# NetSys/demi

Hardware: AMD Instinct MI355X
Metric: candidate schedules evaluated/sec on Raft-5 fuzz (RandomScheduler executions) (higher is better)
Workload: dtype u8

## Files before the change

demi_amd/_native.py:

```python
import ctypes as C
import os

from . import types as T

_HERE = os.path.dirname(os.path.abspath(__file__))
LIB_PATH = os.path.join(_HERE, "libdemi_gpu.so")

EXPORTS = ["demi_ctx_create", "demi_ctx_destroy", "demi_last_error", "demi_version", "demi_model_load",
           "demi_trace_load", "demi_random_explore", "demi_random_explore_dev", "demi_random_get_trace", "demi_collect_violations_dev",
           "demi_replay_load", "demi_replay_batch", "demi_replay_batch_dev", "demi_dpor_load", "demi_dpor_batch", "demi_dpor_explore", "demi_random_explore_violations", "demi_random_get_trace_carried",
           "demi_replay_removal_batch", "demi_replay_get_kept", "demi_replay_recorded_len", "demi_ddmin", "demi_dpor_set_traces", "demi_model_specialize", "demi_model_is_specialized", "demi_model_code_id",
           "demi_specialize_check", "demi_specialize_source", "demi_specialize_source_k1", "demi_provenance_prune", "demi_device_probe", "demi_device_probe_mix", "demi_calib_rw", "demi_random_explore_flagged", "demi_collect_flagged_dev", "demi_random_explore_submit", "demi_random_explore_wait", "demi_trace_len",
           "demi_comm_unique_id", "demi_comm_create", "demi_comm_create_host", "demi_comm_destroy", "demi_comm_rank",
           "demi_comm_allgather_dev", "demi_random_explore_sharded", "demi_replay_batch_sharded", "demi_abi_version", "demi_replay_externals_len", "demi_edit_distance_dpor_ddmin", "demi_dpor_explored", "demi_random_ddmin", "demi_random_explore_candidates", "demi_ext_payload_areas",
           "demi_replay_wildcard_load", "demi_replay_wildcard_batch", "demi_replay_wildcard_get_trace",
           "demi_replay_wildcard_candidates", "demi_wildcard_ddmin",
           "demi_fuzz_stride", "demi_fuzz_generate", "demi_random_explore_tests", "demi_fuzz_campaign",
           "demi_fuzz_generate_fields", "demi_random_explore_tests_areas", "demi_fuzz_campaign_fields",
           "demi_fuzz_launch_summary", "demi_fuzz_launch_summary_row", "demi_fuzz_campaign_pipelined",
           "demi_replay_removal_round", "demi_minimize_internals", "demi_replay_wildcard_round", "demi_minimize_wildcards",
           "demi_replay_batch_submit", "demi_replay_batch_wait",
           "demi_dpor_wildcard_batch", "demi_wildcard_dpor_test"]

_lib = None
# ... 131 lines not shown
                                            C.c_void_p, C.c_void_p, C.c_void_p, C.c_void_p]
    L.demi_random_explore_tests_areas.argtypes = [C.c_void_p, C.c_uint64, C.c_void_p, C.c_void_p, C.c_void_p, C.c_uint32, C.c_uint32, C.c_uint32,
                                                  C.POINTER(T.Limits), C.c_void_p, C.c_void_p]
    L.demi_fuzz_campaign_fields.argtypes = [C.c_void_p, C.POINTER(T.FuzzParams), C.POINTER(T.FuzzFieldGen), C.POINTER(T.FuzzCampaignParams),
                                            C.POINTER(T.Limits), C.c_void_p, C.c_void_p, C.c_uint32, C.POINTER(T.FuzzCampaignResult)]
    L.demi_fuzz_launch_summary.argtypes = [C.c_void_p, C.c_void_p, C.c_void_p, C.c_uint32, C.c_uint32, C.POINTER(T.FuzzSummary)]
    L.demi_fuzz_launch_summary_row.argtypes = [C.c_void_p, C.c_void_p, C.c_void_p, C.c_uint32]
    L.demi_fuzz_campaign_pipelined.argtypes = [C.c_void_p, C.POINTER(T.FuzzParams), C.POINTER(T.FuzzFieldGen), C.POINTER(T.FuzzCampaignParams),
                                               C.POINTER(T.FuzzPipelineParams), C.POINTER(T.Limits), C.c_void_p, C.c_void_p, C.c_uint32,
                                               C.POINTER(T.FuzzCampaignResult), C.POINTER(T.FuzzPipelineStats)]
    L.demi_replay_removal_round.argtypes = [C.c_void_p, C.c_void_p, C.c_void_p, C.c_uint32, C.POINTER(T.Limits), C.c_void_p,
                                            C.POINTER(T.RemovalRoundResult)]
    L.demi_minimize_internals.argtypes = [C.c_void_p, C.POINTER(T.Limits), C.POINTER(T.IntminParams), C.c_void_p, C.c_uint32,
                                          C.POINTER(C.c_uint32), C.c_void_p, C.c_uint32, C.c_void_p, C.c_uint32, C.POINTER(T.IntminStats)]
    L.demi_replay_wildcard_round.argtypes = [C.c_void_p, C.c_void_p, C.c_void_p, C.c_uint32, C.POINTER(T.Limits), C.c_void_p,
                                             C.POINTER(T.WildcardRoundResult)]
    L.demi_minimize_wildcards.argtypes = [C.c_void_p, C.POINTER(T.Limits), C.POINTER(T.WcminParams), C.c_void_p, C.c_uint32,
                                          C.POINTER(C.c_uint32), C.c_void_p, C.c_uint32, C.c_void_p, C.c_uint32, C.POINTER(T.WcminStats)]
    for name in EXPORTS:
        fn = getattr(L, name)
        assert fn.argtypes is not None or name in ("demi_version",), "no argtypes for %s" % name
    _lib = L
    return L


def specialize_check(model_struct):
    log = C.create_string_buffer(4096)
    n = lib().demi_specialize_check(C.byref(model_struct), log, len(log))
    if n < 0:
        raise DemiError(n, log.value.decode(errors="replace"))
    return int(n), log.value.decode()


def specialize_source(model_struct, k1=False):
    buf = C.create_string_buffer(1 << 20)
    n = (lib().demi_specialize_source_k1 if k1 else lib().demi_specialize_source)(C.byref(model_struct), buf, len(buf))
    if n < 0:
        raise DemiError(n, buf.value.decode(errors="replace"))
    return buf.value.decode()


class Context:

    def __init__(self, device=0):
        self._h = C.c_void_p()
        rc = lib().demi_ctx_create(device, C.byref(self._h))
        if rc != 0:
            raise DemiError(rc, "demi_ctx_create failed (no MI355X visible? the GPU path has no CPU fallback)")
        self.device = device

    def close(self):
        if self._h:
            lib().demi_ctx_destroy(self._h)
            self._h = C.c_void_p()

    def __del__(self):
        try:
            self.close()
        except Exception:
            pass

    def _check(self, rc):
        if rc != 0:
            raise DemiError(rc, lib().demi_last_error(self._h).decode())

    def model_load(self, model_struct):
        self._check(lib().demi_model_load(self._h, C.byref(model_struct)))

    def model_specialize(self, enable=True):
# ... 715 lines not shown
```

demi_amd/csrc/demi_gpu.hip:

```cpp
#include <hip/hip_runtime.h>

#include <cstdarg>
#include <cstdio>
#include <cstring>
#include <algorithm>
#include <memory>
#include <new>
#include <queue>
#include <string>
#include <type_traits>
#include <unordered_map>
#include <unordered_set>
#include <vector>
#include <chrono>

#include "../../include/demi_gpu.h"
#include "knobs.hpp"
#include "devbuf.hpp"
#include "k1_random_explore.hpp"
#include "k2_replay.hpp"
#include "k2_removal_round.hpp"
#include "k2_wildcard.hpp"
#include "k2_wildcard_cand.hpp"
#include "k2_wildcard_round.hpp"
// ... 610 lines not shown
           h.n_timer_types, h.timer_types, (unsigned long long)h.tix_packed, h.n_msg_types);
  src = defs + src;
  if (h.inv_kind & DEMI_INV_PROGRAM) src = "#define DEMI_JIT_INV_PROG 1\n" + src;
  if (h.wide) src = "#define DEMI_WIDE 1\n" + src;
  if (is_big(h)) {
    uint32_t type_of_tix = 0;
    for (uint32_t t = 0; t < h.n_msg_types; t++) if ((h.timer_types >> t) & 1u) type_of_tix |= t << (5u * (h.meta[t] >> 8));
    src = "#define DEMI_BIG 1\n#define DEMI_JIT_TYPE_OF_TIX " + std::to_string(type_of_tix) + "u\n" + src;
  }
  if (kernel == JK_K3W) src = "#define DEMI_K3_DECLS_ONLY 1\n" + src;
  src = demi_jit::tq_defines(h) + src;
  src = demi_jit::init_hits_define(h) + src;
  if (h.npay > 2) src = "#define DEMI_JIT_NPAY " + std::to_string(h.npay) + "\n" + src;
  if (h.arr_len) src = "#define DEMI_JIT_ARR_LEN " + std::to_string(h.arr_len) + "u\n" + src;
  {
    bool crash = false, rnd = false;
    for (uint32_t pc = 0; pc < h.code_len; pc++) { crash |= (h.code[pc] & 0xFFu) == DEMI_OP_CRASH; rnd |= (h.code[pc] & 0x3Fu) == DEMI_OP_RND; }
    if (!crash) src = "#define DEMI_JIT_NO_CRASH 1\n" + src;
    if (!rnd) src = "#define DEMI_JIT_NO_RND 1\n" + src;
  }
  if (const char* d = demi_host::knob("DEMI_JIT_DEFINES")) {
    std::string extra, item;
    for (const char* c = d;; c++) {
      if (*c == ';' || *c == '\0') {
        if (!item.empty()) { const size_t eq = item.find('='); extra += "#define " + (eq == std::string::npos ? item : item.substr(0, eq) + " " + item.substr(eq + 1)) + "\n"; }
        item.clear();
        if (*c == '\0') break;
      } else item += *c;
    }
    src = extra + src;
  }
  if (const long x = demi_host::knob_int("DEMI_JIT_K1_WAVES_PER_EU", 1, 8, 0))
    src = "#define DEMI_K1_MIN_WAVES_PER_EU " + std::to_string(x) + "\n" + src;
  src += demi_jit::generate_vm(h, jk_is_k1(kernel) && !jk_k1_records(kernel) && !demi_host::knob("DEMI_JIT_NO_FX_SCHED"));
  src += "#define DEMI_VM_RUN vm_run_jit\n#include \"";
  src += kJit[kernel].include;
  src += "\"\n";
  if (kJit[kernel].args) src += std::string("template __global__ void ") + kJit[kernel].name + "(const " + kJit[kernel].args + ");\n";
  return src;
}

static int jit_compile(demi_ctx* ctx, const DevModel& h, int kernel, std::vector<char>& image, std::string& name) {
#ifdef DEMI_NO_JIT_SOURCES
  return fail(ctx, DEMI_ERR_DEVICE, "specialisation failed: this library was built without the embedded kernel sources "
                                    "(build it with __graft_entry__.build())");
#endif
  static demi_jit::Rtc rtc;
  std::vector<demi_jit::Header> headers(kJitHeaders, kJitHeaders + sizeof(kJitHeaders) / sizeof(kJitHeaders[0]));
  std::vector<std::string> lowered;
  std::string err;
  std::string source = jit_source(h, kernel);
#ifdef DEMI_K1_PHASES
  source = "#define DEMI_K1_PHASES 1\n" + source;
#endif
  if (const char* dump = demi_host::knob("DEMI_JIT_DUMP_SRC")) {
    if (FILE* f = fopen((std::string(dump) + "." + std::to_string(kernel)).c_str(), "w")) { fputs(source.c_str(), f); fclose(f); }
  }
  const char* level = (jk_is_k1(kernel) && !jk_k1_records(kernel)) ? "-Os" : "-O3";
  if (!demi_jit::compile(rtc, source, headers, {kJit[kernel].name}, image, lowered, err, level))
    return fail(ctx, DEMI_ERR_DEVICE, "specialisation failed: %s", err.c_str());
  name = lowered[0];
  if (const char* dump = demi_host::knob("DEMI_JIT_DUMP")) {
    if (FILE* f = fopen((std::string(dump) + "." + std::to_string(kernel)).c_str(), "wb")) { fwrite(image.data(), 1, image.size(), f); fclose(f); }
  }
  return DEMI_OK;
}

static uint64_t code_object_text_hash(const std::vector<char>& image) {
  const unsigned char* b = reinterpret_cast<const unsigned char*>(image.data());
  size_t lo = 0, hi = image.size();
  auto rd = [&](size_t off, int bytes) -> uint64_t {
    uint64_t v = 0;
    for (int i = 0; i < bytes; i++) v |= (uint64_t)b[off + i] << (8 * i);
    return v;
  };
  if (image.size() > 64 && b[0] == 0x7F && b[1] == 'E' && b[2] == 'L' && b[3] == 'F' && b[4] == 2) {
    const uint64_t shoff = rd(0x28, 8), shentsize = rd(0x3A, 2), shnum = rd(0x3C, 2), shstrndx = rd(0x3E, 2);
    if (shentsize >= 64 && shstrndx < shnum && shoff + shnum * shentsize <= image.size()) {
      const uint64_t stroff = rd(shoff + shstrndx * shentsize + 0x18, 8), strsize = rd(shoff + shstrndx * shentsize + 0x20, 8);
      for (uint64_t i = 0; i < shnum; i++) {
        const uint64_t sh = shoff + i * shentsize, name = rd(sh, 4), off = rd(sh + 0x18, 8), size = rd(sh + 0x20, 8);
        if (name + 6 <= strsize && stroff + name + 6 <= image.size() && !memcmp(b + stroff + name, ".text", 6) &&
            off + size <= image.size()) { lo = off; hi = off + size; }
      }
    }
  }
  uint64_t h = 0xCBF29CE484222325ULL;
  for (size_t i = lo; i < hi; i++) h = (h ^ b[i]) * 0x100000001B3ULL;
  return h ? h : 1;
}

static int jit_load(demi_ctx* ctx, int k) {
  std::vector<char> image;
  std::string name;
  int rc = jit_compile(ctx, ctx->hmodel, k, image, name);
  if (rc) return rc;
  if (k == JK_K1) ctx->jit_code_id = code_object_text_hash(image);
  if (jk_is_k1(k) && !jk_k1_records(k)) ctx->jit_k1_fxq_slots = demi_jit::k1_fxq_slots(ctx->hmodel, !demi_host::knob("DEMI_JIT_NO_FX_SCHED"));
  HIP_TRY(ctx, hipSetDevice(ctx->device));
  hipError_t e = hipModuleLoadData(&ctx->jit_module[k], image.data());
  if (e != hipSuccess) { ctx->jit_module[k] = nullptr; return fail(ctx, DEMI_ERR_DEVICE, "hipModuleLoadData: %s", hipGetErrorString(e)); }
  e = hipModuleGetFunction(&ctx->jit_fn[k], ctx->jit_module[k], name.c_str());
  if (e != hipSuccess) {
    (void)hipModuleUnload(ctx->jit_module[k]);
    ctx->jit_module[k] = nullptr; ctx->jit_fn[k] = nullptr;
    return fail(ctx, DEMI_ERR_DEVICE, "hipModuleGetFunction(%s): %s", name.c_str(), hipGetErrorString(e));
  }
  return DEMI_OK;
}

static hipFunction_t jit_kernel(demi_ctx* ctx, int k) {
  if (!ctx->jit_enabled) return nullptr;
  if (!ctx->jit_fn[k] && !ctx->jit_failed[k]) {
    const std::string keep = ctx->err;
    if (jit_load(ctx, k) != DEMI_OK) { ctx->jit_failed[k] = true; ctx->jit_why = ctx->err; ctx->err = keep; }
  }
  return ctx->jit_fn[k];
}

static bool compiled_only(const DevModel& h) { return h.wide != 0 || h.arr_len != 0; }
static bool jit_table_runs_in(const DevModel& h, int k) {
  const unsigned f = kJit[k].flags;
  return !(f & (compiled_only(h) ? JF_NARROW_ONLY : JF_WIDE_ONLY)) && !((f & JF_NO_BIG) && is_big(h)) &&
         !((f & JF_NO_PAYLOADS) && h.npay > 2) && !((f & JF_NO_ARRAY) && h.arr_len);
}
static int need_compiled(demi_ctx* ctx, hipFunction_t jit, const char* what) {
  if (!compiled_only(ctx->hmodel) || jit) return DEMI_OK;
  const std::string why = ctx->jit_enabled ? ctx->jit_why : std::string("not specialised");
  return fail(ctx, DEMI_ERR_INVALID_MODEL, "a DEMI_MODEL_WIDE model runs only as a compiled table: demi_model_specialize must succeed first (%s: %s)", what, why.c_str());
}

// ... 67 lines not shown
      const char* rk = demi_host::knob("DEMI_SPECIALIZE_CHECK_ROUND");
      const bool is_r = (kJit[k].flags & JF_ROUND) != 0;
      if (is_r ? !rk : (rk && !strcmp(rk, "only"))) continue;
    }
    {
      const char* wk = demi_host::knob("DEMI_SPECIALIZE_CHECK_K3W");
      const bool is_w = (kJit[k].flags & JF_K3W) != 0;
      if (is_w ? !wk : (wk && !strcmp(wk, "only"))) continue;
    }
    if (k != JK_K1 && demi_host::knob("DEMI_SPECIALIZE_CHECK_K1_ONLY")) continue;
    rc = jit_compile(&tmp, *h, k, image, name);
    total += (long)image.size();
    names += (k ? " " : "") + name;
  }
  if (log && log_cap) { snprintf(log, log_cap, "%s", rc ? tmp.err.c_str() : names.c_str()); }
  return rc ? (long)rc : total;
}

extern "C" long demi_specialize_source(const demi_model* m, char* out, size_t cap) {
  demi_ctx tmp;
  auto h = std::make_unique<DevModel>();
  int rc = build_host_model(&tmp, m, *h);
  if (rc) { if (out && cap) snprintf(out, cap, "%s", tmp.err.c_str()); return (long)rc; }
  const std::string src = demi_jit::generate_vm(*h);
  if (out && cap) snprintf(out, cap, "%s", src.c_str());
  return (long)src.size();
}

extern "C" long demi_specialize_source_k1(const demi_model* m, char* out, size_t cap) {
  demi_ctx tmp;
  auto h = std::make_unique<DevModel>();
  int rc = build_host_model(&tmp, m, *h);
  if (rc) { if (out && cap) snprintf(out, cap, "%s", tmp.err.c_str()); return (long)rc; }
  const std::string src = demi_jit::generate_vm(*h, true);
  if (out && cap) snprintf(out, cap, "%s", src.c_str());
  return (long)src.size();
}

static int upload_ext_areas(demi_ctx* ctx, const demi_ext_event* ev, uint32_t n, uint64_t* d_events);
extern "C" int demi_trace_load(demi_ctx* ctx, const demi_ext_event* events, uint32_t n_events) {
  if (!ctx) return DEMI_ERR_INVALID_ARG;
  if (!ctx->have_model) return fail(ctx, DEMI_ERR_NO_MODEL, "demi_model_load must precede demi_trace_load");
  if (!events && n_events) return fail(ctx, DEMI_ERR_INVALID_ARG, "null events");
  int rc = validate_trace(ctx, ctx->hmodel, events, n_events);
  if (rc) return rc;
  rc = quiesce(ctx);
  if (rc) return rc;
  ctx->trace.assign(events, events + n_events);
  ctx->started_mask = 0;
  ctx->n_batches = 1;
  for (uint32_t i = 0; i < n_events; i++) {
    if (events[i].kind == DEMI_EV_START) ctx->started_mask |= 1u << events[i].a;
    if (events[i].kind == DEMI_EV_WAIT_QUIESCENCE) ctx->n_batches++;
  }
  static_assert(sizeof(demi_ext_event) == 8, "event is one 8-byte word");
  HIP_TRY(ctx, hipSetDevice(ctx->device));
  if (n_events)
    HIP_TRY(ctx, hipMemcpy(ctx->d_trace, events, sizeof(demi_ext_event) * n_events, hipMemcpyHostToDevice));
  rc = upload_ext_areas(ctx, events, n_events, ctx->d_trace);
  if (rc) return rc;
  ctx->have_trace = true;
  return DEMI_OK;
}

extern "C" int demi_ext_payload_areas(demi_ctx* ctx, const uint64_t* areas, uint32_t n) {
  if (!ctx) return DEMI_ERR_INVALID_ARG;
  ctx->have_staged_areas = false;
// ... 3934 lines not shown
```

demi_amd/csrc/jit.hpp:

```cpp
#pragma once
#include "knobs.hpp"

#include <dlfcn.h>

#include <algorithm>
#include <cstdio>
#include <cstdlib>
#include <cstring>
#include <string>
#include <vector>

#include "sim_core.hpp"

namespace demi_jit {

struct FxSchedule {
  bool ok = false;
  std::vector<uint32_t> cls;
  std::vector<int32_t> slot;
};
enum : uint32_t { FXK_SEND = 0, FXK_CANCEL = 1, FXK_TSET = 2, FXK_CRASH = 3 };
inline uint32_t fx_class_of(uint32_t row) {
  const uint32_t op = row & 0x3Fu, type = (row >> 17) & 0x7Fu;
  if (op == DEMI_OP_SEND || op == DEMI_OP_BCAST) return FXK_SEND << 16;
  if (op == DEMI_OP_TCANCEL) return (FXK_CANCEL << 16) | (op << 8) | type;
  if (op == DEMI_OP_TSET || op == DEMI_OP_TREP) return (FXK_TSET << 16) | (op << 8) | type;
  return FXK_CRASH << 16;
}
inline FxSchedule fx_schedule(const demi::DevModel& h) {
  using namespace demi;
  FxSchedule S;
  const uint32_t n = h.code_len;
  S.slot.assign(n, -1);
  auto succ = [&](uint32_t pc, uint32_t out[2]) -> int {
    const uint32_t row = h.code[pc], cw = op_control(row & 0x3Fu);
    auto clip = [&](uint32_t t) { return t < n ? t : n; };
    if (cw & CW_HALT) return 0;
    if (cw & CW_IF) { out[0] = clip(pc + 1); out[1] = clip(pc + 1 + ((row >> 17) & 0x7Fu)); return 2; }
    if (cw & (CW_SKIPZ | CW_SKIPNZ)) { out[0] = clip(pc + 1); out[1] = clip(pc + 1 + (row >> 24)); return 2; }
    if (cw & CW_SKIP) { out[0] = clip(pc + 1 + (row >> 24)); return 1; }
    out[0] = clip(pc + 1);
    return 1;
  };
  auto is_fx = [&](uint32_t pc) { return (op_control(h.code[pc] & 0x3Fu) & CW_FX) != 0; };
  std::vector<uint32_t> starts;
  for (uint32_t i = 0; i < h.n_classes * h.n_msg_types; i++) {
    const uint32_t st = h.handler_start[i];
    if (st == 0xFFFF || st >= n) continue;
    if (std::find(starts.begin(), starts.end(), st) == starts.end()) starts.push_back(st);
  }
  std::vector<uint32_t> most(n + 1, 0);
  for (uint32_t pc = n; pc-- > 0;) {
    uint32_t o[2], m = 0;
    const int k = succ(pc, o);
    for (int i = 0; i < k; i++) m = std::max(m, most[o[i]]);
    most[pc] = m + (is_fx(pc) ? 1u : 0u);
  }
  for (uint32_t st : starts) if (most[st] > DEMI_FX_CAP) return S;
  std::vector<std::vector<uint32_t>> seqs;
  {
    size_t budget = 20000;
    std::vector<uint32_t> cur;
    struct Frame { uint32_t pc; int next; size_t depth; };
    for (uint32_t st : starts) {
      std::vector<Frame> stack;
      stack.push_back({st, 0, 0});
      cur.clear();
      while (!stack.empty() && budget) {
        Frame& f = stack.back();
        if (f.pc >= n) {
          if (!cur.empty() && std::find(seqs.begin(), seqs.end(), cur) == seqs.end()) seqs.push_back(cur);
          budget--;
          stack.pop_back();
          continue;
        }
        uint32_t o[2];
        const int k = succ(f.pc, o);
        if (f.next == 0) {
          f.depth = cur.size();
          if (is_fx(f.pc)) cur.push_back(fx_class_of(h.code[f.pc]));
          if (k == 0) {
            if (!cur.empty() && std::find(seqs.begin(), seqs.end(), cur) == seqs.end()) seqs.push_back(cur);
            budget--;
          }
        }
        if (f.next < k) {
          const uint32_t to = o[f.next];
          f.next++;
          cur.resize(f.depth + (is_fx(f.pc) ? 1 : 0));
          stack.push_back({to, 0, 0});
        } else {
          cur.resize(f.depth);
          stack.pop_back();
        }
      }
    }
  }
  auto weight = [](uint32_t c) -> uint32_t { const uint32_t k = c >> 16; return k == FXK_TSET ? 2u : (k == FXK_CRASH ? 1u : 4u); };
  {
    std::vector<size_t> at(seqs.size(), 0);
    for (;;) {
      std::vector<std::pair<uint32_t, uint32_t>> votes;
      for (size_t i = 0; i < seqs.size(); i++) {
        if (at[i] >= seqs[i].size()) continue;
        const uint32_t c = seqs[i][at[i]];
        bool hit = false;
        for (auto& v : votes) if (v.first == c) { v.second++; hit = true; }
        if (!hit) votes.push_back({c, 1u});
      }
      if (votes.empty()) break;
      uint32_t best = 0;
      for (uint32_t i = 1; i < votes.size(); i++) if (votes[i].second > votes[best].second) best = i;
      const uint32_t c = votes[best].first;
      S.cls.push_back(c);
      for (size_t i = 0; i < seqs.size(); i++) if (at[i] < seqs[i].size() && seqs[i][at[i]] == c) at[i]++;
      if (S.cls.size() > 4 * DEMI_FX_CAP) return S;
    }
    uint32_t best_cost = 0;
    for (uint32_t c : S.cls) best_cost += weight(c);
    size_t nodes = 200000;
    std::vector<uint32_t> cur;
    std::vector<size_t> pos(seqs.size(), 0);
    struct Rec {
      const std::vector<std::vector<uint32_t>>& seqs; std::vector<uint32_t>& best; uint32_t& best_cost; size_t& nodes;
      decltype(weight)& w;
      void go(std::vector<size_t>& pos, std::vector<uint32_t>& cur, uint32_t cost) {
        if (nodes == 0) return;
        nodes--;
        std::vector<uint32_t> fronts;
        uint32_t need = 0;
        for (size_t i = 0; i < seqs.size(); i++) {
          if (pos[i] >= seqs[i].size()) continue;
          if (std::find(fronts.begin(), fronts.end(), seqs[i][pos[i]]) == fronts.end()) fronts.push_back(seqs[i][pos[i]]);
          uint32_t rest = 0;
          for (size_t k = pos[i]; k < seqs[i].size(); k++) rest += w(seqs[i][k]);
          need = std::max(need, rest);
        }
        if (fronts.empty()) {
          if (cost < best_cost || (cost == best_cost && cur.size() < best.size())) { best = cur; best_cost = cost; }
          return;
        }
        if (cost + need > best_cost || (cost + need == best_cost && cur.size() + 1 >= best.size())) return;
        for (uint32_t c : fronts) {
          std::vector<size_t> saved = pos;
          for (size_t i = 0; i < seqs.size(); i++) if (pos[i] < seqs[i].size() && seqs[i][pos[i]] == c) pos[i]++;
          cur.push_back(c);
          go(pos, cur, cost + w(c));
          cur.pop_back();
          pos = saved;
        }
      }
    } rec{seqs, S.cls, best_cost, nodes, weight};
    rec.go(pos, cur, 0);
  }
  std::vector<int32_t> lo(n + 1, -1);
  for (uint32_t st : starts) lo[st] = 0;
  for (uint32_t pc = 0; pc < n; pc++) {
    if (lo[pc] < 0) continue;
    int32_t next = lo[pc];
    if (is_fx(pc)) {
      const uint32_t c = fx_class_of(h.code[pc]);
      int32_t j = next;
      while (j < (int32_t)S.cls.size() && S.cls[j] != c) j++;
      if (j >= (int32_t)S.cls.size()) { S.cls.push_back(c); j = (int32_t)S.cls.size() - 1; }
      S.slot[pc] = j;
      next = j + 1;
    }
    uint32_t o[2];
    const int k = succ(pc, o);
    for (int i = 0; i < k; i++) if (o[i] < n) lo[o[i]] = std::max(lo[o[i]], next);
  }
  {
    std::vector<int32_t> used(S.cls.size(), 0), remap(S.cls.size(), -1);
    for (uint32_t pc = 0; pc < n; pc++) if (S.slot[pc] >= 0) used[S.slot[pc]] = 1;
    std::vector<uint32_t> cls2;
    for (size_t j = 0; j < S.cls.size(); j++) if (used[j]) { remap[j] = (int32_t)cls2.size(); cls2.push_back(S.cls[j]); }
    for (uint32_t pc = 0; pc < n; pc++) if (S.slot[pc] >= 0) S.slot[pc] = remap[S.slot[pc]];
    S.cls.swap(cls2);
  }
  S.ok = S.cls.size() <= DEMI_FX_CAP;
  return S;
}

inline uint32_t k1_fxq_slots(const demi::DevModel& h, bool sched) {
  if (!sched) return DEMI_FX_CAP;
  const FxSchedule fxs = fx_schedule(h);
  if (!fxs.ok) return DEMI_FX_CAP;
  uint32_t nq = 0;
  for (uint32_t c : fxs.cls) nq += (c >> 16) == FXK_SEND;
  return nq ? nq : 1u;
}

inline std::string tq_defines(const demi::DevModel& h) {
  if (h.n_actors > DEMI_MAX_ACTORS || h.n_timer_types == 0 || h.n_actors * h.n_timer_types > 16) return "";
  uint32_t type_of_tix = 0;
  for (uint32_t t = 0; t < h.n_msg_types; t++)
    if ((h.timer_types >> t) & 1u) type_of_tix |= t << (5u * ((h.meta[t] >> 8) & 3u));
  char buf[64];
  snprintf(buf, sizeof buf, "#define DEMI_JIT_TQ4_TYPES 0x%xu\n", type_of_tix);
  return buf;
}

inline std::string init_hits_define(const demi::DevModel& h) {
  if ((h.inv_kind & DEMI_INV_PROGRAM) || h.inv_fa >= 8u) return "";
  const bool big = h.n_actors > DEMI_MAX_ACTORS;
  uint32_t hits = 0;
  for (uint32_t a = 0; a < h.n_actors; a++) {
    const uint32_t f = h.inv_fa;
    uint32_t v;
    if (big || h.wide) v = (uint32_t)((big ? h.init_state_big : h.init_state_wide)[2 * a + (f >> 2)] >> (16 * (f & 3))) & 0xFFFFu;
    else v = (uint32_t)(h.init_state[a] >> (8 * f)) & 0xFFu;
    hits |= (uint32_t)(((h.inv_kind & 0xFFu) == DEMI_INV_AGREE) ? (v != 0) : (v == h.inv_va)) << a;
  }
  char buf[64];
  snprintf(buf, sizeof buf, "#define DEMI_JIT_INIT_HITS 0x%xu\n", hits);
  return buf;
}

inline std::string generate_vm(const demi::DevModel& h, bool sched = false) {
  using namespace demi;
  std::string s;
  char buf[512];
  auto emit = [&](const char* fmt, auto... a) { snprintf(buf, sizeof buf, fmt, a...); s += buf; };
  FxSchedule fxs;
  std::vector<uint32_t> fxq_of_slot;
  if (sched) fxs = fx_schedule(h);
  if (fxs.ok) {
    s += "#define DEMI_JIT_FX_SCHED 1\n#define DEMI_JIT_FX_APPLY";
    uint32_t nq = 0;
    for (size_t j = 0; j < fxs.cls.size(); j++) {
      const uint32_t c = fxs.cls[j], type = c & 0xFFu;
      const bool snd = (c >> 16) == FXK_SEND;
      emit(" DEMI_FX_SLOT(%zu, %uu, %uu, %uu, %uu, %uu)", j, c >> 16, (c >> 8) & 0xFFu, type, snd ? 0u : (h.meta[type & 31u] >> 8), snd ? nq : 0u);
      fxq_of_slot.push_back(snd ? nq : 0u);
      if (snd) nq++;
    }
    emit("\n#define DEMI_JIT_FXQ_SLOTS %uu\n", nq ? nq : 1u);
  }
  s += "namespace demi {\n";
  const bool long_msg = h.npay > 2;
  const char* fx_pack_fn = long_msg ? "fx_pack_area" : "fx_pack";
  if (fxs.ok)
    s += std::string("#define DEMI_FX_AT(SLOT, Q, OP, TYPE, TGT, ...) { mem.fxq[(Q) * 64] = ") + fx_pack_fn + "(OP, TYPE, TGT, __VA_ARGS__); nfx |= 1u << (SLOT); }\n"
         "#define DEMI_FX_MARK(SLOT) { nfx |= 1u << (SLOT); }\n";
  else
    s += std::string("#define DEMI_FX(OP, TYPE, TGT, ...) { if (nfx >= DEMI_FX_CAP) { flags |= DEMI_V_QUEUE_OVF; goto done; } "
         "mem.fxq[nfx * 64] = ") + fx_pack_fn + "(OP, TYPE, TGT, __VA_ARGS__); nfx++; }\n";
  const bool wide = h.wide != 0;
  const unsigned RM = wide ? 65535u : 255u, SM = wide ? 15u : 7u;
  emit("__device__ inline uint32_t vm_run_jit(const Tables& t, const LaneMem& mem, %s w, uint32_t& flags, uint64_t& app_rng) {\n",
       wide ? "word_t" : "uint32_t");
  s += "  const uint32_t type = w_type(w), me = w_dst(w);\n";
  s += "  const uint32_t entry = t.hs[((t.ac_packed >> (4 * me)) & 15u) * t.NT + type];\n";
  s += "  if (entry == 0xFFFFu) return 0;\n";
  if (wide) {
    s += "  const uint64_t st0 = mem.st[(ST_WORDS * me) * 64], st1 = mem.st[(ST_WORDS * me + 1) * 64];\n";
    s += "  uint32_t r0 = (uint32_t)st0 & 65535u, r1 = (uint32_t)(st0 >> 16) & 65535u, r2 = (uint32_t)(st0 >> 32) & 65535u, "
         "r3 = (uint32_t)(st0 >> 48) & 65535u,\n           r4 = (uint32_t)st1 & 65535u, r5 = (uint32_t)(st1 >> 16) & 65535u, "
         "r6 = (uint32_t)(st1 >> 32) & 65535u, r7 = (uint32_t)(st1 >> 48) & 65535u;\n";
  } else {
    s += "  const uint64_t st0 = mem.st[(ST_WORDS * me) * 64];\n";
    s += "  uint32_t r0 = (uint32_t)st0 & 255u, r1 = (uint32_t)(st0 >> 8) & 255u, r2 = (uint32_t)(st0 >> 16) & 255u, "
         "r3 = (uint32_t)(st0 >> 24) & 255u,\n           r4 = (uint32_t)(st0 >> 32) & 255u, r5 = (uint32_t)(st0 >> 40) & 255u, "
         "r6 = (uint32_t)(st0 >> 48) & 255u, r7 = (uint32_t)(st0 >> 56) & 255u;\n";
  }
  s += "  uint32_t r8 = 0, r9 = 0, r10 = 0, r11 = 0, r12 = w_p0(w), r13 = w_p1(w), r14 = w_src(w), r15 = me;\n";
  s += "  uint32_t nfx = 0;\n";
  s += "  (void)r8; (void)r9; (void)r10; (void)r11; (void)r12; (void)r13; (void)r14; (void)r15;\n";
  if (long_msg) s += "  uint32_t q2 = 0, q3 = 0, q4 = 0, q5 = 0;   // DEMI_OP_PSET: the staged payload fields of the messages sent next\n"
                     "  (void)q2; (void)q3; (void)q4; (void)q5;\n";
  std::vector<uint32_t> starts;
  for (uint32_t i = 0; i < h.n_classes * h.n_msg_types; i++) {
    const uint32_t st = h.handler_start[i];
    if (st == 0xFFFF || st >= h.code_len) continue;
    bool seen = false;
    for (uint32_t x : starts) seen |= (x == st);
    if (!seen) starts.push_back(st);
// ... 71 lines not shown
    snprintf(d, sizeof d, "r%u", dsti);
    if (bimm) snprintf(b, sizeof b, "%uu", braw); else snprintf(b, sizeof b, "r%u", braw & 15u);
    emit("  L%u: ", pc);
    const uint32_t cw = op_control(op);
    if ((cw & CW_HALT) && !(cw & CW_FX)) {
      s += "goto done;\n";
      continue;
    }
    if (cw & CW_ALU) {
      char val[96];
      alu_value(op, a, b, val, sizeof val);
      if (pred_of[pc] >= 0) emit("%s = c%d ? (%s) : %s;\n", d, pred_of[pc], val, d);
      else emit("%s = %s;\n", d, val);
    } else if (cw & CW_IF) {
      if (pc + 1 < h.code_len && pred_of[pc + 1] == (int32_t)pc)
        emit("c%u = (%s %s %s);\n", pc, a, relop[op - DEMI_OP_IFEQ], b);
      else
        emit("if (!(%s %s %s)) goto %s;\n", a, relop[op - DEMI_OP_IFEQ], b, target(pc + 1 + aux).c_str());
    } else if (cw & CW_SKIPZ) {
      emit("if (%s == 0u) goto %s;\n", a, target(pc + 1 + braw).c_str());
    } else if (cw & CW_SKIPNZ) {
      emit("if (%s != 0u) goto %s;\n", a, target(pc + 1 + braw).c_str());
    } else if (cw & CW_SKIP) {
      emit("goto %s;\n", target(pc + 1 + braw).c_str());
    } else if (cw & CW_STX) {
      emit("arr_store(mem.st, me, %s, %s);\n", b, a);
    } else if (cw & CW_PSET) {
      emit("q%u = %s;\n", aux >= 2 && aux <= 5 ? aux : 2u, b);
    } else {
      char pay[96];
      if (long_msg) snprintf(pay, sizeof pay, "pay_area(%s, %s, q2, q3, q4, q5)", d, b);
      else snprintf(pay, sizeof pay, "%s, %s", d, b);
      if (fxs.ok && (fxs.cls[fxs.slot[pc]] >> 16) != FXK_SEND)
        emit("DEMI_FX_MARK(%d)%s\n", fxs.slot[pc], (cw & CW_HALT) ? " goto done;" : "");
      else if (fxs.ok)
        emit("DEMI_FX_AT(%d, %uu, %uu, %uu, %s > FX_NOBODY ? FX_NOBODY : %s, %s)\n", fxs.slot[pc], fxq_of_slot[fxs.slot[pc]], row & 0xFFu, aux, a, a, pay);
      else
        emit("DEMI_FX(%uu, %uu, %s > FX_NOBODY ? FX_NOBODY : %s, %s)%s\n", row & 0xFFu, aux, a, a, pay, (cw & CW_HALT) ? " goto done;" : "");
    }
  }
  s += "  done:\n";
  if (wide)
    s += "  mem.st[(ST_WORDS * me) * 64] = (uint64_t)(r0 | (r1 << 16)) | ((uint64_t)(r2 | (r3 << 16)) << 32);\n"
         "  mem.st[(ST_WORDS * me + 1) * 64] = (uint64_t)(r4 | (r5 << 16)) | ((uint64_t)(r6 | (r7 << 16)) << 32);\n";
  else
    s += "  mem.st[(ST_WORDS * me) * 64] = (uint64_t)(r0 | (r1 << 8) | (r2 << 16) | (r3 << 24)) | "
         "((uint64_t)(r4 | (r5 << 8) | (r6 << 16) | (r7 << 24)) << 32);\n";
  s += "  return nfx;\n}\n";
  if (h.inv_kind & DEMI_INV_PROGRAM) {
    s += "__device__ inline uint32_t inv_prog_jit(const uint64_t* st, uint32_t actor, uint32_t& key, uint32_t exists, uint32_t n_actors) {\n"
         "  (void)exists; (void)n_actors;\n";
    if (wide) {
      s += "  const uint64_t st0 = st[(ST_WORDS * actor) * 64], st1 = st[(ST_WORDS * actor + 1) * 64];\n";
      s += "  uint32_t r0 = (uint32_t)st0 & 65535u, r1 = (uint32_t)(st0 >> 16) & 65535u, r2 = (uint32_t)(st0 >> 32) & 65535u, "
           "r3 = (uint32_t)(st0 >> 48) & 65535u,\n           r4 = (uint32_t)st1 & 65535u, r5 = (uint32_t)(st1 >> 16) & 65535u, "
           "r6 = (uint32_t)(st1 >> 32) & 65535u, r7 = (uint32_t)(st1 >> 48) & 65535u;\n";
    } else {
      s += "  const uint64_t st0 = st[(ST_WORDS * actor) * 64];\n";
      s += "  uint32_t r0 = (uint32_t)st0 & 255u, r1 = (uint32_t)(st0 >> 8) & 255u, r2 = (uint32_t)(st0 >> 16) & 255u, "
           "r3 = (uint32_t)(st0 >> 24) & 255u,\n           r4 = (uint32_t)(st0 >> 32) & 255u, r5 = (uint32_t)(st0 >> 40) & 255u, "
           "r6 = (uint32_t)(st0 >> 48) & 255u, r7 = (uint32_t)(st0 >> 56) & 255u;\n";
    }
    s += "  uint32_t r8 = 0, r9 = 0, r10 = 0, r11 = 0, r12 = 0, r13 = 0, r14 = 0, r15 = actor;\n";
    s += "  (void)r0; (void)r1; (void)r2; (void)r3; (void)r4; (void)r5; (void)r6; (void)r7; (void)r10; (void)r11; (void)r12; (void)r13; (void)r14; (void)r15;\n";
    auto itarget = [&](uint32_t pc) -> std::string { return pc >= h.code_len ? "idone" : "I" + std::to_string(pc); };
    arr_of = "st, actor";
    for (uint32_t pc = h.inv_fa; pc < h.code_len; pc++) {
// ... 135 lines not shown
```

demi_amd/csrc/k1_random_explore.hpp:

```cpp
#pragma once

#include "sim_core.hpp"

#ifndef DEMI_VM_RUN
#define DEMI_VM_RUN vm_run
#endif

namespace demi {

struct K1Args {
  const DevModel* model;
  const uint64_t* trace;
  uint32_t n_ev;
  uint32_t exists;
  uint64_t seed_base;
  const uint64_t* seeds;
  uint64_t n;
  uint32_t max_messages, interval, looking_for_valid, looking_for;
  demi_verdict* out;
  unsigned long long* work_counter;
  uint32_t p_max;
  uint32_t* spill;
  demi_rec_event* rec_out;
  uint32_t* rec_count;
// ... 405 lines not shown
#endif
  uint32_t hits = 0;
  word_t lastw = 0;
#ifdef DEMI_K1_NO_LASTW
#define LASTW() pend_load(mem, n_pend - 1)
#define LASTW_SET(W) do {} while (0)
#define LASTW_RELOAD() do {} while (0)
#else
#define LASTW() lastw
#define LASTW_SET(W) do { lastw = (W); } while (0)
#define LASTW_RELOAD() do { if (n_pend != 0) lastw = pend_load(mem, n_pend - 1); } while (0)
#endif
  uint32_t next_id = 1, n_rec = 0;
  demi_rec_event* rec = nullptr;

  uint64_t b_next = 0, b_end = 0;
  bool exhausted = false;

#define REC_PUSH(KIND, SND, RCV, TYPE, AREA, FL, EXT, ID)   \
  do {                                                                                        \
    if (REC) {                                                                                \
      if (n_rec < args.rec_cap) {                                                             \
        demi_rec_event e_;                                                                    \
        e_.kind = (uint8_t)(KIND); e_.snd = (uint8_t)(SND); e_.rcv = (uint8_t)(RCV);          \
        const uint64_t ar_ = (uint64_t)(AREA);                                                \
        e_.msg_type = (uint8_t)(TYPE); e_.p0 = (uint16_t)ar_; e_.p1 = (uint16_t)(ar_ >> 16);  \
        e_.flags = (uint8_t)(FL); e_.ext_idx = (uint8_t)(EXT); e_.p_hi = (uint16_t)(ar_ >> 32); e_.id = (ID); \
        rec[n_rec] = e_;                                                                      \
      }                                                                                       \
      n_rec++;                                                                                \
    }                                                                                         \
  } while (0)

#define PEND_APPEND(WORD, ID, TD_ENTRY)                               \
  do {                                                                \
    if (n_pend + n_norm >= PMAX) { flags |= DEMI_V_PENDING_OVF; }     \
    else {                                                            \
      pend_store(mem, n_pend, (WORD));                                \
      LASTW_SET(WORD);                                                \
      if (REC) aux_store(mem, n_pend, (ID));                          \
      if ((TD_ENTRY) >= 0) {                                          \
        unsigned char* const p_ = td_ptr((uint32_t)(TD_ENTRY));       \
        *p_ = (unsigned char)((*p_ == TD_NONE) ? n_pend : TD_MANY);   \
      }                                                               \
      n_pend++;                                                       \
    }                                                                 \
  } while (0)

#define NORM_APPEND(WORD, ID)                                         \
  do {                                                                \
    if (n_pend + n_norm >= PMAX) { flags |= DEMI_V_PENDING_OVF; }     \
    else {                                                            \
      const word_t w_ = (WORD);                                       \
      const uint32_t pr_ = w_src(w_) * MAX_ACT + w_dst(w_);           \
      norm_store(n_norm, w_);                                         \
      if (REC) norm_aux_store(n_norm, (ID));                          \
      if (!pair_has(pr_)) { pair_set(n_pairs, pr_); n_pairs++; if (!BIG_TU) pairmask |= 1ull << pr_; } \
      n_norm++;                                                       \
    }                                                                 \
  } while (0)

#define TIMER_BIT(RCV, TYPE) ((tmask_t)1 << ((RCV) * DEMI_MAX_TIMER_TYPES + tix_of(TYPE)))

  auto enqueue_timer = [&](uint32_t rcv, uint32_t type, tmask_t tbit) {
    const uint32_t b = TimerQ::pack(rcv, type, (BIG_TU || TQ_NARROW) ? tix_of(type) : 0u);
    if (just & tbit) {
      if (n_resend >= DEMI_RESEND_CAP) { flags |= DEMI_V_QUEUE_OVF; return; }
      resend.push(n_resend, b);
      n_resend++;
    } else {
      if (n_tq >= DEMI_TQ_CAP) { flags |= DEMI_V_QUEUE_OVF; return; }
      tq.push(n_tq, b);
      n_tq++;
      if (INQ) inq |= tbit;
    }
  };

  auto pend_remove_moved = [&](uint32_t idx, word_t lw) {
    const uint32_t last = n_pend - 1;
    pend_store(mem, idx, lw);
    if (REC) aux_store(mem, idx, aux_load(mem, last));
    uint32_t e;
    if (idx != last && timer_entry(lw, e)) { unsigned char* const p = td_ptr(e); if (*p == last) *p = (unsigned char)idx; }
    n_pend = last;
// ... 567 lines not shown
#else
            *p = (unsigned char)TD_NONE;
            pend_remove_moved(d, LASTW());
#endif
          } else {
            uint32_t first = 0xFFFFFFFFu, second = 0xFFFFFFFFu, copies = 0;
            for (uint32_t q = 0; q < n_pend; q++)
              if (pend_load(mem, q) == wantw) {
                if (copies == 0) first = q; else if (copies == 1) second = q;
                copies++;
              }
            if (copies != 0) {
              const uint32_t last = n_pend - 1;
#ifdef DEMI_K1_NO_RM_KNOWN
              pend_remove(first, wantw, LASTW());
#else
              pend_remove_moved(first, LASTW());
#endif
              if (copies == 2) *p = (unsigned char)(second == last ? first : second);
            }
            if (copies <= 1) *p = (unsigned char)TD_NONE;
          }
        }
      }
    };
    auto apply_timer_set = [&](bool repeating, uint32_t type, tmask_t bit) {
      if (!(rep & bit)) {
        if (repeating) rep |= bit;
        enqueue_timer(me, type, bit);
      }
    };
    if (deliver) {
#ifdef DEMI_JIT_FX_SCHED
#define DEMI_FX_SLOT(J, KIND, OP, TYPE, TIDX, Q)                                                                      \
      if (((nfx >> (J)) & 1u) && !(flags & DEMI_OVF_ANY)) {                                                           \
        if ((KIND) == 0u) apply_send(mem.fxq[(Q) * 64]);                      \
        else if ((KIND) == 1u) apply_cancel((TYPE), (tmask_t)1 << (me * DEMI_MAX_TIMER_TYPES + (TIDX)), (TIDX));               \
        else if ((KIND) == 2u) apply_timer_set((OP) == DEMI_OP_TREP, (TYPE), (tmask_t)1 << (me * DEMI_MAX_TIMER_TYPES + (TIDX))); \
        else if (CRASHES) blocked |= 1u << me;                                                                        \
      }                                                                                                               \
      PH_MARK((KIND) == 0u ? 6 : (KIND) == 1u ? 7 : 8);
      DEMI_JIT_FX_APPLY
#undef DEMI_FX_SLOT
#else
      for (uint32_t k = 0; k < nfx && !(flags & DEMI_OVF_ANY); k++) {
        const word_t fxw = mem.fxq[k * 64];
        const uint32_t fx = (uint32_t)fxw;
        const uint32_t op = fx & 31u, type = (fx >> 5) & 31u;
        PH_MARK(9);
        if (op <= DEMI_OP_BCAST) { apply_send(fxw); PH_MARK(6); }
        else if (op == DEMI_OP_CRASH) { if (CRASHES) blocked |= 1u << me; }
        else if (op == DEMI_OP_TCANCEL) { apply_cancel(type, TIMER_BIT(me, type), tix_of(type)); PH_MARK(7); }
        else { apply_timer_set(op == DEMI_OP_TREP, type, TIMER_BIT(me, type)); PH_MARK(8); }
      }
#endif
      if (!REBIN && (flags & DEMI_OVF_ANY)) ph = PH_FINISH;
    }
    if (REBIN) {
      if (deliver) {
        uint32_t* const xb = rb_x + rb_owner;
        uint32_t k = 0;
        xb[k++ * RB_WG] = (flags & 0xFu) | (n_pend << 4) | (n_tq << 12) | (n_resend << 16) | (rb_hit << 28);
        xb[k++ * RB_WG] = (uint32_t)lastw; if (WIDE_TU) xb[k++ * RB_WG] = (uint32_t)((uint64_t)lastw >> 32);
        xb[k++ * RB_WG] = (uint32_t)tq.bits; xb[k++ * RB_WG] = (uint32_t)((uint64_t)tq.bits >> 32);
        xb[k++ * RB_WG] = (uint32_t)resend.bits; xb[k++ * RB_WG] = (uint32_t)((uint64_t)resend.bits >> 32);
        xb[k++ * RB_WG] = just; xb[k++ * RB_WG] = rep;
        if (RB_CRASHES) xb[k++ * RB_WG] = blocked;
        if (APP_RND) { xb[k++ * RB_WG] = (uint32_t)app_rng; xb[k++ * RB_WG] = (uint32_t)(app_rng >> 32); }
// ... 6 lines not shown
        flags = pk & 0xFu; n_pend = (pk >> 4) & 0xFFu; n_tq = (pk >> 12) & 0xFu; n_resend = (pk >> 16) & 0xFu;
        { uint64_t lw = xi[j++ * RB_WG]; if (WIDE_TU) lw |= (uint64_t)xi[j++ * RB_WG] << 32; lastw = (word_t)lw; }
        tq.bits = (TimerQ::bits_t)(xi[j * RB_WG] | ((uint64_t)xi[(j + 1) * RB_WG] << 32)); j += 2;
        resend.bits = (TimerQ::bits_t)(xi[j * RB_WG] | ((uint64_t)xi[(j + 1) * RB_WG] << 32)); j += 2;
        just = xi[j++ * RB_WG]; rep = xi[j++ * RB_WG];
        if (RB_CRASHES) blocked = xi[j++ * RB_WG];
        if (APP_RND) { app_rng = xi[j * RB_WG] | ((uint64_t)xi[(j + 1) * RB_WG] << 32); j += 2; }
        if (rb_me != 0xFFu) {
          hits = (hits & ~(1u << rb_me)) | (((pk >> 28) & 1u) << rb_me);
          if (flags & DEMI_OVF_ANY) ph = PH_FINISH;
        }
      }
      mem = own_mem; st = own_mem.st; tdir = own_tdir;
      if (batch_no != 0) {
        const uint32_t* bt = s_batch + (size_t)(batch_no - 1) * K1_BATCH_WORDS;
        reach = (uint64_t)bt[7] | ((uint64_t)bt[8] << 32);
      }
      rb_it ^= 1u;
    }

    PH_MARK(9);
  }
#ifdef DEMI_K1_PHASES
  PH_MARK(11);
  if (lane == 0 && args.phase_out) {
    unsigned long long* o = args.phase_out + ((size_t)blockIdx.x * K1_WAVES + wave) * 16;
    for (int i = 0; i < 12; i++) o[i] = ph_t[i];
    o[14] = ph_iters; o[15] = ph_active;
  }
#endif
#undef PH_MARK
#undef REC_PUSH
#undef PEND_APPEND
#undef NORM_APPEND
#undef LASTW
#undef LASTW_SET
#undef LASTW_RELOAD
#undef TIMER_BIT
}

}
```

Measured before the change: 345.7 million.

## Let JIT effect scheduler reorder commuting timer-set and send effects

```diff
diff --git a/demi_amd/_native.py b/demi_amd/_native.py
--- a/demi_amd/_native.py
+++ b/demi_amd/_native.py
@@ -187,9 +187,22 @@
     return int(n), log.value.decode()
 
 
-def specialize_source(model_struct, k1=False):
-    buf = C.create_string_buffer(1 << 20)
-    n = (lib().demi_specialize_source_k1 if k1 else lib().demi_specialize_source)(C.byref(model_struct), buf, len(buf))
+def specialize_source(model_struct, k1=False, fx_commute=False):
+    saved = {k: os.environ.get(k) for k in ("DEMI_EXPERIMENT", "DEMI_JIT_NO_FX_COMMUTE")}
+    try:
+        if k1 and not fx_commute:
+            os.environ["DEMI_EXPERIMENT"] = "1"
+            os.environ["DEMI_JIT_NO_FX_COMMUTE"] = "1"
+        elif k1:
+            os.environ.pop("DEMI_JIT_NO_FX_COMMUTE", None)
+        buf = C.create_string_buffer(1 << 20)
+        n = (lib().demi_specialize_source_k1 if k1 else lib().demi_specialize_source)(C.byref(model_struct), buf, len(buf))
+    finally:
+        for k, v in saved.items():
+            if v is None:
+                os.environ.pop(k, None)
+            else:
+                os.environ[k] = v
     if n < 0:
         raise DemiError(n, buf.value.decode(errors="replace"))
     return buf.value.decode()
diff --git a/demi_amd/csrc/demi_gpu.hip b/demi_amd/csrc/demi_gpu.hip
--- a/demi_amd/csrc/demi_gpu.hip
+++ b/demi_amd/csrc/demi_gpu.hip
@@ -666,7 +666,8 @@
   }
   if (const long x = demi_host::knob_int("DEMI_JIT_K1_WAVES_PER_EU", 1, 8, 0))
     src = "#define DEMI_K1_MIN_WAVES_PER_EU " + std::to_string(x) + "\n" + src;
-  src += demi_jit::generate_vm(h, jk_is_k1(kernel) && !jk_k1_records(kernel) && !demi_host::knob("DEMI_JIT_NO_FX_SCHED"));
+  src += demi_jit::generate_vm(h, jk_is_k1(kernel) && !jk_k1_records(kernel) && !demi_host::knob("DEMI_JIT_NO_FX_SCHED"),
+                               !demi_host::knob("DEMI_JIT_NO_FX_COMMUTE"));
   src += "#define DEMI_VM_RUN vm_run_jit\n#include \"";
   src += kJit[kernel].include;
   src += "\"\n";
@@ -730,7 +731,7 @@
   int rc = jit_compile(ctx, ctx->hmodel, k, image, name);
   if (rc) return rc;
   if (k == JK_K1) ctx->jit_code_id = code_object_text_hash(image);
-  if (jk_is_k1(k) && !jk_k1_records(k)) ctx->jit_k1_fxq_slots = demi_jit::k1_fxq_slots(ctx->hmodel, !demi_host::knob("DEMI_JIT_NO_FX_SCHED"));
+  if (jk_is_k1(k) && !jk_k1_records(k)) ctx->jit_k1_fxq_slots = demi_jit::k1_fxq_slots(ctx->hmodel, !demi_host::knob("DEMI_JIT_NO_FX_SCHED"), !demi_host::knob("DEMI_JIT_NO_FX_COMMUTE"));
   HIP_TRY(ctx, hipSetDevice(ctx->device));
   hipError_t e = hipModuleLoadData(&ctx->jit_module[k], image.data());
   if (e != hipSuccess) { ctx->jit_module[k] = nullptr; return fail(ctx, DEMI_ERR_DEVICE, "hipModuleLoadData: %s", hipGetErrorString(e)); }
@@ -864,7 +865,7 @@
   auto h = std::make_unique<DevModel>();
   int rc = build_host_model(&tmp, m, *h);
   if (rc) { if (out && cap) snprintf(out, cap, "%s", tmp.err.c_str()); return (long)rc; }
-  const std::string src = demi_jit::generate_vm(*h, true);
+  const std::string src = demi_jit::generate_vm(*h, true, !demi_host::knob("DEMI_JIT_NO_FX_COMMUTE"));
   if (out && cap) snprintf(out, cap, "%s", src.c_str());
   return (long)src.size();
 }
diff --git a/demi_amd/csrc/jit.hpp b/demi_amd/csrc/jit.hpp
--- a/demi_amd/csrc/jit.hpp
+++ b/demi_amd/csrc/jit.hpp
@@ -18,6 +18,8 @@
   bool ok = false;
   std::vector<uint32_t> cls;
   std::vector<int32_t> slot;
+  std::vector<uint8_t> moved;
+  bool any_moved() const { return std::find(moved.begin(), moved.end(), (uint8_t)1) != moved.end(); }
 };
 enum : uint32_t { FXK_SEND = 0, FXK_CANCEL = 1, FXK_TSET = 2, FXK_CRASH = 3 };
 inline uint32_t fx_class_of(uint32_t row) {
@@ -27,11 +29,18 @@
   if (op == DEMI_OP_TSET || op == DEMI_OP_TREP) return (FXK_TSET << 16) | (op << 8) | type;
   return FXK_CRASH << 16;
 }
-inline FxSchedule fx_schedule(const demi::DevModel& h) {
+inline bool fx_commute(uint32_t a, uint32_t b) {
+  const uint32_t ka = a >> 16, kb = b >> 16;
+  return (ka == FXK_TSET && kb == FXK_SEND) || (ka == FXK_SEND && kb == FXK_TSET);
+}
+inline FxSchedule fx_schedule_search(const demi::DevModel& h, bool commute, std::vector<uint8_t> pinned = {}) {
   using namespace demi;
   FxSchedule S;
   const uint32_t n = h.code_len;
   S.slot.assign(n, -1);
+  S.moved.assign(n, 0);
+  pinned.resize(n, 0);
+  auto free_tset = [&](uint32_t pc) { return commute && !pinned[pc] && (fx_class_of(h.code[pc]) >> 16) == FXK_TSET; };
   auto succ = [&](uint32_t pc, uint32_t out[2]) -> int {
     const uint32_t row = h.code[pc], cw = op_control(row & 0x3Fu);
     auto clip = [&](uint32_t t) { return t < n ? t : n; };
@@ -57,8 +66,7 @@
     most[pc] = m + (is_fx(pc) ? 1u : 0u);
   }
   for (uint32_t st : starts) if (most[st] > DEMI_FX_CAP) return S;
-  std::vector<std::vector<uint32_t>> seqs;
-  {
+  auto each_path = [&](auto&& fn) -> bool {
     size_t budget = 20000;
     std::vector<uint32_t> cur;
     struct Frame { uint32_t pc; int next; size_t depth; };
@@ -69,7 +77,7 @@
       while (!stack.empty() && budget) {
         Frame& f = stack.back();
         if (f.pc >= n) {
-          if (!cur.empty() && std::find(seqs.begin(), seqs.end(), cur) == seqs.end()) seqs.push_back(cur);
+          fn(cur);
           budget--;
           stack.pop_back();
           continue;
@@ -78,9 +86,9 @@
         const int k = succ(f.pc, o);
         if (f.next == 0) {
           f.depth = cur.size();
-          if (is_fx(f.pc)) cur.push_back(fx_class_of(h.code[f.pc]));
+          if (is_fx(f.pc)) cur.push_back(f.pc);
           if (k == 0) {
-            if (!cur.empty() && std::find(seqs.begin(), seqs.end(), cur) == seqs.end()) seqs.push_back(cur);
+            fn(cur);
             budget--;
           }
         }
@@ -94,8 +102,25 @@
           stack.pop_back();
         }
       }
-    }
-  }
+      if (!stack.empty()) return false;
+    }
+    return true;
+  };
+  std::vector<std::vector<uint32_t>> seqs;
+  const bool all_paths = each_path([&](const std::vector<uint32_t>& path) {
+    if (path.empty()) return;
+    std::vector<uint32_t> rows = path, q;
+    if (commute)
+      for (size_t i = 0; i < rows.size();) {
+        size_t e = i;
+        while (e < rows.size() && (free_tset(rows[e]) || (fx_class_of(h.code[rows[e]]) >> 16) == FXK_SEND)) e++;
+        std::stable_partition(rows.begin() + i, rows.begin() + e, [&](uint32_t pc) { return free_tset(pc); });
+        i = e + 1;
+      }
+    for (uint32_t pc : rows) q.push_back(fx_class_of(h.code[pc]));
+    if (std::find(seqs.begin(), seqs.end(), q) == seqs.end()) seqs.push_back(q);
+  });
+  if (commute && !all_paths) return fx_schedule_search(h, false);
   auto weight = [](uint32_t c) -> uint32_t { const uint32_t k = c >> 16; return k == FXK_TSET ? 2u : (k == FXK_CRASH ? 1u : 4u); };
   {
     std::vector<size_t> at(seqs.size(), 0);
@@ -153,22 +178,49 @@
     } rec{seqs, S.cls, best_cost, nodes, weight};
     rec.go(pos, cur, 0);
   }
-  std::vector<int32_t> lo(n + 1, -1);
+  std::vector<int32_t> lo(n + 1, -1), lo_t(n + 1, 0);
   for (uint32_t st : starts) lo[st] = 0;
   for (uint32_t pc = 0; pc < n; pc++) {
     if (lo[pc] < 0) continue;
-    int32_t next = lo[pc];
+    int32_t next = lo[pc], next_t = lo_t[pc];
     if (is_fx(pc)) {
-      const uint32_t c = fx_class_of(h.code[pc]);
-      int32_t j = next;
+      const uint32_t c = fx_class_of(h.code[pc]), kind = c >> 16;
+      int32_t j = free_tset(pc) ? next_t : next;
       while (j < (int32_t)S.cls.size() && S.cls[j] != c) j++;
       if (j >= (int32_t)S.cls.size()) { S.cls.push_back(c); j = (int32_t)S.cls.size() - 1; }
       S.slot[pc] = j;
-      next = j + 1;
+      next = std::max(next, j + 1);
+      if (kind != FXK_SEND) next_t = std::max(next_t, j + 1);
     }
     uint32_t o[2];
     const int k = succ(pc, o);
-    for (int i = 0; i < k; i++) if (o[i] < n) lo[o[i]] = std::max(lo[o[i]], next);
+    for (int i = 0; i < k; i++) if (o[i] < n) { lo[o[i]] = std::max(lo[o[i]], next); lo_t[o[i]] = std::max(lo_t[o[i]], next_t); }
+  }
+  if (commute) {
+    bool good = true, pins = false;
+    each_path([&](const std::vector<uint32_t>& rows) {
+      for (size_t j = 0; j < rows.size(); j++)
+        for (size_t i = 0; i < j; i++) {
+          const uint32_t ci = fx_class_of(h.code[rows[i]]), cj = fx_class_of(h.code[rows[j]]);
+          const int32_t si = S.slot[rows[i]], sj = S.slot[rows[j]];
+          if (si < sj) continue;
+          if (fx_commute(ci, cj) && free_tset(rows[j]) && si != sj) S.moved[rows[j]] = 1;
+          else good = false;
+        }
+    });
+    each_path([&](const std::vector<uint32_t>& rows) {
+      bool has_moved = false, exact = true;
+      for (uint32_t pc : rows) has_moved |= S.moved[pc] != 0;
+      if (!has_moved) return;
+      for (size_t j = 0; j < rows.size(); j++) {
+        if ((fx_class_of(h.code[rows[j]]) >> 16) != FXK_TSET) continue;
+        for (size_t i = j + 1; i < rows.size(); i++)
+          if ((fx_class_of(h.code[rows[i]]) >> 16) == FXK_SEND && S.slot[rows[i]] > S.slot[rows[j]]) exact = false;
+      }
+      if (!exact) for (uint32_t pc : rows) if (S.moved[pc]) { pinned[pc] = 1; pins = true; }
+    });
+    if (!good) return fx_schedule_search(h, false);
+    if (pins) return fx_schedule_search(h, true, pinned);
   }
   {
     std::vector<int32_t> used(S.cls.size(), 0), remap(S.cls.size(), -1);
@@ -182,9 +234,18 @@
   return S;
 }
 
-inline uint32_t k1_fxq_slots(const demi::DevModel& h, bool sched) {
+inline FxSchedule fx_schedule(const demi::DevModel& h, bool commute = true) {
+  const FxSchedule plain = fx_schedule_search(h, false);
+  if (!commute) return plain;
+  const FxSchedule moved = fx_schedule_search(h, true);
+  if (!moved.ok || !moved.any_moved()) return plain;
+  auto cost = [](const FxSchedule& s) { uint32_t c = 0; for (uint32_t x : s.cls) c += (x >> 16) == FXK_TSET ? 2u : ((x >> 16) == FXK_CRASH ? 1u : 4u); return c; };
+  return (!plain.ok || cost(moved) <= cost(plain)) ? moved : plain;
+}
+
+inline uint32_t k1_fxq_slots(const demi::DevModel& h, bool sched, bool commute = true) {
   if (!sched) return DEMI_FX_CAP;
-  const FxSchedule fxs = fx_schedule(h);
+  const FxSchedule fxs = fx_schedule(h, commute);
   if (!fxs.ok) return DEMI_FX_CAP;
   uint32_t nq = 0;
   for (uint32_t c : fxs.cls) nq += (c >> 16) == FXK_SEND;
@@ -217,14 +278,14 @@
   return buf;
 }
 
-inline std::string generate_vm(const demi::DevModel& h, bool sched = false) {
+inline std::string generate_vm(const demi::DevModel& h, bool sched = false, bool commute = true) {
   using namespace demi;
   std::string s;
   char buf[512];
   auto emit = [&](const char* fmt, auto... a) { snprintf(buf, sizeof buf, fmt, a...); s += buf; };
   FxSchedule fxs;
   std::vector<uint32_t> fxq_of_slot;
-  if (sched) fxs = fx_schedule(h);
+  if (sched) fxs = fx_schedule(h, commute);
   if (fxs.ok) {
     s += "#define DEMI_JIT_FX_SCHED 1\n#define DEMI_JIT_FX_APPLY";
     uint32_t nq = 0;
@@ -236,13 +297,19 @@
       if (snd) nq++;
     }
     emit("\n#define DEMI_JIT_FXQ_SLOTS %uu\n", nq ? nq : 1u);
+    if (fxs.any_moved()) {
+      uint32_t mv = 0;
+      for (uint32_t pc = 0; pc < h.code_len; pc++) if (fxs.moved[pc]) mv |= 1u << fxs.slot[pc];
+      emit("#define DEMI_JIT_FX_MOVED_SLOTS 0x%xu\n", mv);
+    }
   }
   s += "namespace demi {\n";
   const bool long_msg = h.npay > 2;
   const char* fx_pack_fn = long_msg ? "fx_pack_area" : "fx_pack";
   if (fxs.ok)
     s += std::string("#define DEMI_FX_AT(SLOT, Q, OP, TYPE, TGT, ...) { mem.fxq[(Q) * 64] = ") + fx_pack_fn + "(OP, TYPE, TGT, __VA_ARGS__); nfx |= 1u << (SLOT); }\n"
-         "#define DEMI_FX_MARK(SLOT) { nfx |= 1u << (SLOT); }\n";
+         "#define DEMI_FX_MARK(SLOT) { nfx |= 1u << (SLOT); }\n"
+         "#define DEMI_FX_MARK_MOVED(SLOT) { nfx |= (1u << (SLOT)) | (DEMI_V_QUEUE_OVF << DEMI_FX_CAP); }\n";
   else
     s += std::string("#define DEMI_FX(OP, TYPE, TGT, ...) { if (nfx >= DEMI_FX_CAP) { flags |= DEMI_V_QUEUE_OVF; goto done; } "
          "mem.fxq[nfx * 64] = ") + fx_pack_fn + "(OP, TYPE, TGT, __VA_ARGS__); nfx++; }\n";
@@ -380,7 +447,7 @@
       if (long_msg) snprintf(pay, sizeof pay, "pay_area(%s, %s, q2, q3, q4, q5)", d, b);
       else snprintf(pay, sizeof pay, "%s, %s", d, b);
       if (fxs.ok && (fxs.cls[fxs.slot[pc]] >> 16) != FXK_SEND)
-        emit("DEMI_FX_MARK(%d)%s\n", fxs.slot[pc], (cw & CW_HALT) ? " goto done;" : "");
+        emit("DEMI_FX_MARK%s(%d)%s\n", fxs.moved[pc] ? "_MOVED" : "", fxs.slot[pc], (cw & CW_HALT) ? " goto done;" : "");
       else if (fxs.ok)
         emit("DEMI_FX_AT(%d, %uu, %uu, %uu, %s > FX_NOBODY ? FX_NOBODY : %s, %s)\n", fxs.slot[pc], fxq_of_slot[fxs.slot[pc]], row & 0xFFu, aux, a, a, pay);
       else
diff --git a/demi_amd/csrc/k1_random_explore.hpp b/demi_amd/csrc/k1_random_explore.hpp
--- a/demi_amd/csrc/k1_random_explore.hpp
+++ b/demi_amd/csrc/k1_random_explore.hpp
@@ -461,9 +461,13 @@
     }                                                                                         \
   } while (0)
 
+#ifndef DEMI_JIT_FX_MOVED_SLOTS
+#define DEMI_JIT_FX_MOVED_SLOTS 0u
+#endif
+#define K1_PENDING_OVF() (flags = DEMI_JIT_FX_MOVED_SLOTS ? ((flags & ~DEMI_V_QUEUE_OVF) | DEMI_V_PENDING_OVF) : (flags | DEMI_V_PENDING_OVF))
 #define PEND_APPEND(WORD, ID, TD_ENTRY)                               \
   do {                                                                \
-    if (n_pend + n_norm >= PMAX) { flags |= DEMI_V_PENDING_OVF; }     \
+    if (n_pend + n_norm >= PMAX) { K1_PENDING_OVF(); }                \
     else {                                                            \
       pend_store(mem, n_pend, (WORD));                                \
       LASTW_SET(WORD);                                                \
@@ -478,7 +482,7 @@
 
 #define NORM_APPEND(WORD, ID)                                         \
   do {                                                                \
-    if (n_pend + n_norm >= PMAX) { flags |= DEMI_V_PENDING_OVF; }     \
+    if (n_pend + n_norm >= PMAX) { K1_PENDING_OVF(); }                \
     else {                                                            \
       const word_t w_ = (WORD);                                       \
       const uint32_t pr_ = w_src(w_) * MAX_ACT + w_dst(w_);           \
@@ -1112,8 +1116,13 @@
     };
     if (deliver) {
 #ifdef DEMI_JIT_FX_SCHED
+#ifdef DEMI_K1_FX_DROP_MOVED
+      const uint32_t fx_send_stop = DEMI_OVF_ANY;
+#else
+      const uint32_t fx_send_stop = DEMI_JIT_FX_MOVED_SLOTS ? (DEMI_OVF_ANY ^ (nfx >> DEMI_FX_CAP)) : DEMI_OVF_ANY;
+#endif
 #define DEMI_FX_SLOT(J, KIND, OP, TYPE, TIDX, Q)                                                                      \
-      if (((nfx >> (J)) & 1u) && !(flags & DEMI_OVF_ANY)) {                                                           \
+      if (((nfx >> (J)) & 1u) && !(flags & ((KIND) == 0u ? fx_send_stop : DEMI_OVF_ANY))) {                            \
         if ((KIND) == 0u) apply_send(mem.fxq[(Q) * 64]);                      \
         else if ((KIND) == 1u) apply_cancel((TYPE), (tmask_t)1 << (me * DEMI_MAX_TIMER_TYPES + (TIDX)), (TIDX));               \
         else if ((KIND) == 2u) apply_timer_set((OP) == DEMI_OP_TREP, (TYPE), (tmask_t)1 << (me * DEMI_MAX_TIMER_TYPES + (TIDX))); \
@@ -1186,6 +1195,7 @@
 #undef PH_MARK
 #undef REC_PUSH
 #undef PEND_APPEND
+#undef K1_PENDING_OVF
 #undef NORM_APPEND
 #undef LASTW
 #undef LASTW_SET
```

Result: faster. 350.6 million (median of 6 runs) (+1.4%).
